# Frikallo/parakeet.cpp

Measured on AMD Instinct MI355X. Metric: RTFx (audio-sec/wall-sec), mel+encoder+TDT decode, tdt-ctc-110m 10s@b64, higher is better.
Workload: dtype f32; 1 GPU; tdt-ctc-110m, batch=64x10s clips per GPU, TDT greedy decode (the loops of 4 consecutive steps driven as one lock-step batch), fp32 (BASELINE configs[1]); parallelism=dp1 (utterance shards, no data-path collective), decode_group=4, decode_loop=phases, decode_overlap=1

## Files before the change

parakeet.cpp_amd/csrc/kernels/gemm.hip:

```cpp
#include "../pk_devmath.h"
#include "kernels.hpp"
#include <cstdio>
#include <cstdlib>
#include "gemm_pipe.hpp"
#include "gemm_bf16.hpp"
#include "gemm_bf16_glds.hpp"

namespace pk {

typedef float f32x16 __attribute__((ext_vector_type(16)));

static constexpr int BK = 32;
static constexpr int LDP = BK + 1;

template <int BM, int BN, int EPI>
__global__ __launch_bounds__(256) void gemm_nt_kernel(GemmArgs g, int tiles_n, int n_tiles) {
    constexpr int WM = BM / 2, WN = BN / 2;
    constexpr int TM = WM / 32, TN = WN / 32;
    constexpr int A_CH = BM * 8 / 256, W_CH = BN * 8 / 256;
    constexpr int NOUT = (EPI == EPI_GLU) ? BN / 2 : BN;
    static_assert(EPI != EPI_GLU || (TN % 2 == 0), "GLU needs an even number of column tiles per wave");
    extern __shared__ __attribute__((aligned(16))) float smem[];

    int bid = blockIdx.x;
    {
        const int q = n_tiles >> 3, r = n_tiles & 7, xcd = bid & 7, idx = bid >> 3;
        bid = (xcd < r ? xcd * (q + 1) : r * (q + 1) + (xcd - r) * q) + idx;
    }
    const int tile_m = bid / tiles_n, tile_n = bid % tiles_n;
    const int m0 = tile_m * BM, n0 = tile_n * NOUT;
    const int tid = threadIdx.x, lane = tid & 63, wave = tid >> 6;
    const int wm = wave >> 1, wn = wave & 1;

    const float *a_src[A_CH];
    const float *w_src[W_CH];
#pragma unroll
    for (int i = 0; i < A_CH; ++i) {
        const int c = tid + 256 * i, row = c >> 3, c4 = c & 7;
        int gr = m0 + row;
        gr = gr < g.M ? gr : g.M - 1;
        a_src[i] = g.A + (int64_t)gr * g.lda + c4 * 4;
    }
#pragma unroll
    for (int i = 0; i < W_CH; ++i) {
        const int c = tid + 256 * i, v = c >> 3, c4 = c & 7;
        int wr;
        if constexpr (EPI == EPI_GLU) {
            constexpr int HT = TN / 2;
            const int vw = v / WN, rem = v % WN, tn = rem >> 5, cc = rem & 31;
            int col = n0 + vw * (WN / 2) + (tn % HT) * 32 + cc;
            col = col < g.N ? col : g.N - 1;
            wr = (tn / HT) * g.N + col;
        } else {
            wr = n0 + v;
            wr = wr < g.N ? wr : g.N - 1;
        }
        w_src[i] = g.W + (int64_t)wr * g.ldw + c4 * 4;
    }

    float4 ra[A_CH], rw[W_CH];
    auto gload = [&](int kt) {
#pragma unroll
        for (int i = 0; i < A_CH; ++i) ra[i] = *reinterpret_cast<const float4 *>(a_src[i] + kt * BK);
#pragma unroll
        for (int i = 0; i < W_CH; ++i) rw[i] = *reinterpret_cast<const float4 *>(w_src[i] + kt * BK);
    };
    auto lstore = [&](int buf) {
        float *As = smem + buf * (BM + BN) * LDP;
        float *Ws = As + BM * LDP;
#pragma unroll
        for (int i = 0; i < A_CH; ++i) {
            const int c = tid + 256 * i;
            float *d = As + (c >> 3) * LDP + (c & 7) * 4;
            d[0] = ra[i].x; d[1] = ra[i].y; d[2] = ra[i].z; d[3] = ra[i].w;
        }
#pragma unroll
        for (int i = 0; i < W_CH; ++i) {
            const int c = tid + 256 * i;
            float *d = Ws + (c >> 3) * LDP + (c & 7) * 4;
            d[0] = rw[i].x; d[1] = rw[i].y; d[2] = rw[i].z; d[3] = rw[i].w;
        }
    };

    f32x16 acc[TM][TN];
#pragma unroll
    for (int i = 0; i < TM; ++i)
#pragma unroll
        for (int j = 0; j < TN; ++j)
#pragma unroll
            for (int r = 0; r < 16; ++r) acc[i][j][r] = 0.0f;

    const int nk = g.K / BK;
    gload(0);
    lstore(0);
    __syncthreads();
    const int frag = (lane & 31) * LDP + (lane >> 5);
    for (int kt = 0; kt < nk; ++kt) {
        const int cur = kt & 1;
        if (kt + 1 < nk) gload(kt + 1);
        const float *Ab = smem + cur * (BM + BN) * LDP + wm * WM * LDP + frag;
        const float *Wb = smem + cur * (BM + BN) * LDP + BM * LDP + wn * WN * LDP + frag;
#pragma unroll
        for (int kk = 0; kk < BK / 2; ++kk) {
            float a[TM], b[TN];
#pragma unroll
            for (int i = 0; i < TM; ++i) a[i] = Ab[i * 32 * LDP + 2 * kk];
#pragma unroll
            for (int j = 0; j < TN; ++j) b[j] = Wb[j * 32 * LDP + 2 * kk];
#pragma unroll
            for (int i = 0; i < TM; ++i)
#pragma unroll
                for (int j = 0; j < TN; ++j)
                    acc[i][j] = __builtin_amdgcn_mfma_f32_32x32x2f32(a[i], b[j], acc[i][j], 0, 0, 0);
        }
        if (kt + 1 < nk) lstore(cur ^ 1);
        __syncthreads();
    }

    const int lc = lane & 31, lr = 4 * (lane >> 5);
    constexpr int TNO = (EPI == EPI_GLU) ? TN / 2 : TN;
#pragma unroll
    for (int j = 0; j < TNO; ++j) {
        const int col = n0 + wn * (EPI == EPI_GLU ? WN / 2 : WN) + j * 32 + lc;
        if (col >= g.N) continue;
        const float bias = g.bias ? g.bias[col] : 0.0f;
        float bias_g = 0.0f;
        if constexpr (EPI == EPI_GLU) bias_g = g.bias ? g.bias[g.N + col] : 0.0f;
#pragma unroll
        for (int i = 0; i < TM; ++i) {
#pragma unroll
            for (int r = 0; r < 16; ++r) {
                const int row = m0 + wm * WM + i * 32 + (r & 3) + 8 * (r >> 2) + lr;
                if (row >= g.M) continue;
                float v = acc[i][j][r];
                if (g.bias) v = v + bias;
                if constexpr (EPI == EPI_RELU) {
                    v = v > 0.0f ? v : 0.0f;
                } else if constexpr (EPI == EPI_SILU) {
                    v = dsiluf(v);
                } else if constexpr (EPI == EPI_RESID) {
                    const float y = v * g.alpha;
                    v = g.resid[(int64_t)row * g.ldr + col] + y;
                } else if constexpr (EPI == EPI_GLU) {
                    float gt = acc[i][j + TN / 2][r];
                    if (g.bias) gt = gt + bias_g;
                    v = v * dsigmoidf(gt);
                }
                if (g.remap_rows) g.out[(int64_t)(row / g.remap_rows) * g.remap_gs + (int64_t)(row % g.remap_rows) * g.remap_rs + (int64_t)col * g.remap_cs] = v;
                else g.out[(int64_t)row * g.ldo + (col < g.sigma_cols ? ((col & ~15) | ((col & 3) << 2) | ((col >> 2) & 3)) : col)] = v;
            }
        }
    }
}

template <int BM, int BN, int EPI>
static void launch_one(const GemmArgs &a, hipStream_t s) {
    constexpr int NOUT = (EPI == EPI_GLU) ? BN / 2 : BN;
    const int tiles_m = (a.M + BM - 1) / BM, tiles_n = (a.N + NOUT - 1) / NOUT;
    const int n_tiles = tiles_m * tiles_n;
    constexpr size_t lds = 2 * (size_t)(BM + BN) * LDP * sizeof(float);
    static DynLdsSlots slots;
    ensure_dyn_lds(slots, reinterpret_cast<const void *>(&gemm_nt_kernel<BM, BN, EPI>), lds);
    hipLaunchKernelGGL((gemm_nt_kernel<BM, BN, EPI>), dim3(n_tiles), dim3(256), lds, s, a, tiles_n, n_tiles);
}

template <int EPI>
static void launch_epi(const GemmArgs &a, hipStream_t s) {
    if (a.K < 64) { launch_one<64, 64, EPI>(a, s); return; }
    const int64_t tiles128 = (int64_t)((a.M + 127) / 128) * ((a.N + 127) / 128);
    if (a.M >= 1024 && a.N >= 256 && a.K >= 1024 && a.K % 64 == 0 && tiles128 <= 256) { launch_gemm_pipe<2, 4, 2, 1, 32, EPI, 1>(a, s); return; }
    if constexpr (EPI == EPI_NONE || EPI == EPI_RELU || EPI == EPI_SILU) {
        if (a.ln_stats) { launch_gemm_pipe<4, 2, 1, 2, 32, EPI, 1, true>(a, s); return; }
    }
    if (a.M >= 1024 && (a.N >= 1024 || (a.M >= 65536 && a.N >= 256))) launch_gemm_pipe<4, 2, 1, 2, 32, EPI, 1>(a, s);
    else if (a.M >= 1024 && a.N >= 256 && a.K >= 1024) launch_gemm_pipe<2, 2, 2, 1, 32, EPI>(a, s);
    else if (a.M >= 1024 && a.N >= 256) launch_gemm_pipe<4, 2, 1, 2, 32, EPI, 1>(a, s);
    else launch_gemm_pipe<2, 2, 1, 1, 32, EPI>(a, s);
}

void launch_gemm_smallm(const GemmArgs &a, int epi, hipStream_t s);

bool gemm_ln_stats_applies(const GemmArgs &a, int epi) {
    if (!a.ln_g || !a.ln_b || !a.ln_stats || a.a_bf16 || a.out_bf16 || a.fast_act || a.a_sigma || a.W_sig) return false;
    if (a.M <= kSmallMRows || a.K < 64 || a.K % 32 != 0 || (a.lda & 3) != 0 || (a.ldw & 3) != 0) return false;
    if (epi == EPI_GLU) return true;
    if (epi != EPI_NONE && epi != EPI_RELU && epi != EPI_SILU) return false;
    const int64_t tiles128 = (int64_t)((a.M + 127) / 128) * ((a.N + 127) / 128);
    if (a.K >= 1024 && a.K % 64 == 0 && tiles128 <= 256 && a.N >= 256) return false;
    return a.M >= 1024 && a.N >= 1024;
}

void launch_gemm(const GemmArgs &a, int epi, hipStream_t s) {
    if (a.ln_stats && !gemm_ln_stats_applies(a, epi)) { fprintf(stderr, "parakeet_amd: internal error: GemmArgs::ln_stats on a product the tile kernel does not fold it into\n"); abort(); }
    if (a.M <= kSmallMRows && a.K % 64 == 0) { launch_gemm_smallm(a, epi, s); return; }
    switch (epi) {
    case EPI_NONE: launch_epi<EPI_NONE>(a, s); break;
    case EPI_RELU: launch_epi<EPI_RELU>(a, s); break;
    case EPI_SILU: launch_epi<EPI_SILU>(a, s); break;
    case EPI_RESID: launch_epi<EPI_RESID>(a, s); break;
    case EPI_GLU:
        if (a.K < 64) launch_one<128, 128, EPI_GLU>(a, s);
        else if (a.ln_stats) launch_gemm_pipe<4, 2, 1, 2, 32, EPI_GLU, 1, true>(a, s);
        else launch_gemm_pipe<4, 2, 1, 2, 32, EPI_GLU, 1>(a, s);
        break;
    default: break;
    }
}


static bool bf16_glds_rule(int M, int N, int K) {
    return M >= 8192 && N >= 512 && K >= 128 && (int64_t)N * K >= (int64_t)1024 * 1024 && (N & 3) == 0;
}
bool gemm_bf16_blocked_handoff(int M, int N, int K, int epi, bool producer) {
    if (!bf16_glds_rule(M, N, K) || (N % 16) != 0 || (K % 64) != 0) return false;
    if (!producer) return true;
    return epi != EPI_RESID && (int64_t)(M + 31) * N < ((int64_t)1 << 31);
}
[[noreturn]] static void bf16_layout_bug(const char *what) {
    fprintf(stderr, "parakeet_amd: internal error: %s (GemmArgs::out_blocked / a_blocked on a kernel that does not implement it)\n", what);
    abort();
}

template <int EPI, bool A16>
static void launch_bf16_epi(const GemmArgs &a, hipStream_t s) {
    if constexpr (A16) {
        if (a.M >= 8192 && a.N >= 512 && a.K >= 128 && (a.lda % 8) == 0 && (a.ldw % 8) == 0 && a.remap_rows == 0 && (a.ldo & 3) == 0 && (a.N & 3) == 0 &&
            (int64_t)a.N * a.K >= (int64_t)1024 * 1024) {
            constexpr int NOUT = (EPI == EPI_GLU) ? 128 : 256;
            auto est = [&](int R) {
                const int64_t tiles = (int64_t)((a.M + R - 1) / R) * ((a.N + NOUT - 1) / NOUT);
                return (double)((tiles + 255) / 256) * ((double)R * a.K * 1.008e-4 + 12.0);
            };
            if (est(192) < est(256)) launch_gemm_bf16_glds<2, 4, 3, 2, EPI>(a, s);
            else launch_gemm_bf16_glds<4, 2, 2, 4, EPI>(a, s);
            return;
        }
    }
    if (a.out_blocked || a.a_blocked) bf16_layout_bug("blocked activation layout requested for the register-staged bf16 kernel");
    if constexpr (EPI == EPI_GLU) {
        launch_gemm_bf16_t<4, 2, 1, 2, EPI_GLU, A16>(a, s);
    } else {
        if (a.M >= 1024 && (a.N >= 1024 || (a.M >= 65536 && a.N >= 256))) launch_gemm_bf16_t<4, 2, 1, 2, EPI, A16>(a, s);
        else if (a.M >= 1024 && a.N >= 256) launch_gemm_bf16_t<2, 2, 2, 1, EPI, A16>(a, s);
        else launch_gemm_bf16_t<2, 2, 1, 1, EPI, A16>(a, s);
    }
}
template <bool A16>
static void launch_gemm_bf16_a(const GemmArgs &a, int epi, hipStream_t s) {
    switch (epi) {
    case EPI_NONE: launch_bf16_epi<EPI_NONE, A16>(a, s); break;
    case EPI_RELU: launch_bf16_epi<EPI_RELU, A16>(a, s); break;
    case EPI_SILU: launch_bf16_epi<EPI_SILU, A16>(a, s); break;
    case EPI_RESID: launch_bf16_epi<EPI_RESID, A16>(a, s); break;
    case EPI_GLU: launch_bf16_epi<EPI_GLU, A16>(a, s); break;
    default: break;
    }
}
void launch_gemm_bf16(const GemmArgs &a, int epi, hipStream_t s) {
    if (gemm_smallm_bf16_applies(a, epi)) { launch_gemm_smallm_bf16(a, epi, s); return; }
    if (a.a_bf16) launch_gemm_bf16_a<true>(a, epi, s);
    else launch_gemm_bf16_a<false>(a, epi, s);
}

double gemm_flops(const GemmArgs &a, int epi) {
    return 2.0 * (double)a.M * (double)a.N * (double)a.K * (epi == EPI_GLU ? 2.0 : 1.0);
}

}
```

parakeet.cpp_amd/csrc/kernels/gemm_pipe.hpp:

```cpp
#ifndef PK_GEMM_PIPE_HPP
#define PK_GEMM_PIPE_HPP
#include <cstdio>
#include <cstdlib>
#include "../pk_devmath.h"
#include "kernels.hpp"

namespace pk {

typedef float gp_f32x16 __attribute__((ext_vector_type(16)));

template <int WGM, int WGN, int TM, int TN, int EPI, int CAP_FLOATS, bool RS_PER_PASS = false, bool EXACT = false>
__device__ __forceinline__ void gp_epilogue(const GemmArgs &g_, gp_f32x16 (&acc)[TM][TN], float *smem, int m0, int n0) {
    struct Flags { int fast_act, out_bf16; };
    const Flags gf{EXACT ? 0 : g_.fast_act, EXACT ? 0 : g_.out_bf16};
    const GemmArgs &g = g_;
    constexpr int NT = 64 * WGM * WGN;
    constexpr int WM = TM * 32, WN = TN * 32, BM = WGM * WM, BN = WGN * WN;
    constexpr int NOUT = (EPI == EPI_GLU) ? BN / 2 : BN;
    const int tid = threadIdx.x, lane = tid & 63, wave = tid >> 6;
    const int wm = wave / WGN, wn = wave % WGN;
    auto epilogue_scalar = [&](int m0, int n0) {
        const int lc = lane & 31, lr = 4 * (lane >> 5);
        constexpr int TNO = (EPI == EPI_GLU) ? TN / 2 : TN;
#pragma unroll
        for (int j = 0; j < TNO; ++j) {
            const int col = n0 + wn * (EPI == EPI_GLU ? WN / 2 : WN) + j * 32 + lc;
            if (col >= g.N) continue;
            const float bias = g.bias ? g.bias[col] : 0.0f;
            float bias_g = 0.0f;
            if constexpr (EPI == EPI_GLU) bias_g = g.bias ? g.bias[g.N + col] : 0.0f;
#pragma unroll
            for (int i = 0; i < TM; ++i) {
#pragma unroll
                for (int r = 0; r < 16; ++r) {
                    const int row = m0 + wm * WM + i * 32 + (r & 3) + 8 * (r >> 2) + lr;
                    if (row >= g.M) continue;
                    float v = acc[i][j][r];
                    if (g.bias) v = v + bias;
                    if constexpr (EPI == EPI_RELU) {
                        v = v > 0.0f ? v : 0.0f;
                    } else if constexpr (EPI == EPI_SILU) {
                        v = gf.fast_act ? fast_siluf(v) : dsiluf(v);
                    } else if constexpr (EPI == EPI_RESID) {
                        const float y = v * g.alpha;
                        v = g.resid[(int64_t)row * g.ldr + col] + y;
                    } else if constexpr (EPI == EPI_GLU) {
                        float gt = acc[i][j + TN / 2][r];
                        if (g.bias) gt = gt + bias_g;
                        v = v * (gf.fast_act ? fast_sigmoidf(gt) : dsigmoidf(gt));
                    }
                    if (g.remap_rows) g.out[(int64_t)(row / g.remap_rows) * g.remap_gs + (int64_t)(row % g.remap_rows) * g.remap_rs + (int64_t)col * g.remap_cs] = v;
                    else g.out[(int64_t)row * g.ldo + (col < g.sigma_cols ? ((col & ~15) | ((col & 3) << 2) | ((col >> 2) & 3)) : col)] = v;
                }
            }
        }
    };
    auto epilogue_wide = [&](int m0, int n0) {
        constexpr int CP = BN + 4;
        constexpr size_t CAP = (size_t)CAP_FLOATS;
        constexpr int NPASS = ((size_t)BM * CP <= CAP) ? 1 : ((size_t)BM / 2 * CP <= CAP && (BM / 2) % 32 == 0) ? 2 : ((size_t)BM / 4 * CP <= CAP && (BM / 4) % 32 == 0) ? 4
                              : ((size_t)BM / 8 * CP <= CAP && (BM / 8) % 32 == 0) ? 8 : BM / 32, PR = BM / NPASS;
        static_assert((size_t)PR * CP <= CAP, "C tile band must fit in the staging buffers");
        static_assert(PR % 32 == 0, "row bands are whole MFMA tiles");
        constexpr int C4 = NOUT / 4, NCH = BM * C4 / NT, RSTEP = NT / C4;
        static_assert((BM * C4) % NT == 0 && NT % C4 == 0, "output tile must split evenly over the threads");
        static_assert(NPASS == 1 || PR % RSTEP == 0, "row bands must split evenly over the threads' row stride");
        const int c4 = tid % C4, rl0 = tid / C4;
        const int col0 = n0 + 4 * c4;
        const bool col_ok = col0 < g.N;
        const bool sig = col0 < g.sigma_cols;
        const int blk = (4 * c4) & ~15, sa = c4 & 3;
        float bs[4] = {0.0f, 0.0f, 0.0f, 0.0f}, bg[4] = {0.0f, 0.0f, 0.0f, 0.0f};
        if (g.bias && col_ok) {
#pragma unroll
            for (int e = 0; e < 4; ++e) {
                bs[e] = g.bias[sig ? n0 + blk + 4 * e + sa : col0 + e];
                if constexpr (EPI == EPI_GLU) bg[e] = g.bias[g.N + col0 + e];
            }
        }
        constexpr int NRS = RS_PER_PASS ? NCH / NPASS : NCH;
        static_assert(!RS_PER_PASS || NCH % NPASS == 0, "chunks must split evenly over the passes");
        float4 rs[NRS];
        if constexpr (EPI == EPI_RESID && !RS_PER_PASS) {
#pragma unroll
            for (int q = 0; q < NCH; ++q) {
                int row = m0 + rl0 + q * RSTEP;
                row = row < g.M ? row : g.M - 1;
                rs[q] = col_ok ? *reinterpret_cast<const float4 *>(g.resid + (int64_t)row * g.ldr + col0) : make_float4(0.0f, 0.0f, 0.0f, 0.0f);
            }
        }
#pragma unroll
        for (int pass = 0; pass < NPASS; ++pass) {
        if constexpr (EPI == EPI_RESID && RS_PER_PASS) {
#pragma unroll
            for (int q = 0; q < NRS; ++q) {
                int row = m0 + rl0 + (pass * NRS + q) * RSTEP;
                row = row < g.M ? row : g.M - 1;
                rs[q] = col_ok ? *reinterpret_cast<const float4 *>(g.resid + (int64_t)row * g.ldr + col0) : make_float4(0.0f, 0.0f, 0.0f, 0.0f);
            }
        }
        __syncthreads();
        {
            const int lc = lane & 31, lr = 4 * (lane >> 5);
#pragma unroll
            for (int i = 0; i < TM; ++i) {
                const int rb = wm * WM + i * 32;
                if (rb / PR != pass) continue;
#pragma unroll
                for (int j = 0; j < TN; ++j)
#pragma unroll
                    for (int r = 0; r < 16; ++r)
                        smem[(rb - pass * PR + (r & 3) + 8 * (r >> 2) + lr) * CP + wn * WN + j * 32 + lc] = acc[i][j][r];
            }
        }
        __syncthreads();
#pragma unroll
        for (int q = 0; q < NCH; ++q) {
            if ((q * RSTEP) / PR != pass) continue;
            const int rl = rl0 + q * RSTEP;
            const int row = m0 + rl;
            const int rs_ = rl - pass * PR;
            float v[4], gt[4];
            if (sig) {
#pragma unroll
                for (int e = 0; e < 4; ++e) v[e] = smem[rs_ * CP + blk + 4 * e + sa];
            } else {
                int vc = 4 * c4;
                if constexpr (EPI == EPI_GLU) vc = (vc / (WN / 2)) * WN + vc % (WN / 2);
                const float4 x = *reinterpret_cast<const float4 *>(smem + rs_ * CP + vc);
                v[0] = x.x; v[1] = x.y; v[2] = x.z; v[3] = x.w;
                if constexpr (EPI == EPI_GLU) {
                    const float4 y = *reinterpret_cast<const float4 *>(smem + rs_ * CP + vc + WN / 2);
                    gt[0] = y.x; gt[1] = y.y; gt[2] = y.z; gt[3] = y.w;
                }
            }
            float rsv[4] = {0.0f, 0.0f, 0.0f, 0.0f};
            if constexpr (EPI == EPI_RESID) { const float4 &rr = rs[RS_PER_PASS ? q - pass * NRS : q]; rsv[0] = rr.x; rsv[1] = rr.y; rsv[2] = rr.z; rsv[3] = rr.w; }
            if (g.bias) {
#pragma unroll
                for (int e = 0; e < 4; ++e) {
                    v[e] = v[e] + bs[e];
                    if constexpr (EPI == EPI_GLU) gt[e] = gt[e] + bg[e];
                }
            }
            if constexpr (EPI == EPI_RELU) {
#pragma unroll
                for (int e = 0; e < 4; ++e) v[e] = v[e] > 0.0f ? v[e] : 0.0f;
            } else if constexpr (EPI == EPI_SILU) {
                if (gf.fast_act) {
#pragma unroll
                    for (int e = 0; e < 4; ++e) v[e] = fast_siluf(v[e]);
                } else {
                    dsilu4(v);
                }
            } else if constexpr (EPI == EPI_RESID) {
#pragma unroll
                for (int e = 0; e < 4; ++e) { const float y = v[e] * g.alpha; v[e] = rsv[e] + y; }
            } else if constexpr (EPI == EPI_GLU) {
                if (gf.fast_act) {
#pragma unroll
                    for (int e = 0; e < 4; ++e) gt[e] = fast_sigmoidf(gt[e]);
                } else {
                    dsigmoid4(gt);
                }
#pragma unroll
                for (int e = 0; e < 4; ++e) v[e] = v[e] * gt[e];
            }
            if (row < g.M && col_ok) {
                if (gf.out_bf16) {
                    typedef __bf16 bf16x4_ __attribute__((ext_vector_type(4)));
                    const bf16x4_ o = {(__bf16)v[0], (__bf16)v[1], (__bf16)v[2], (__bf16)v[3]};
                    *reinterpret_cast<bf16x4_ *>(reinterpret_cast<__bf16 *>(g.out) + (int64_t)row * g.ldo + col0) = o;
                } else {
                    *reinterpret_cast<float4 *>(g.out + (int64_t)row * g.ldo + col0) = make_float4(v[0], v[1], v[2], v[3]);
                }
            }
        }
        }
    };
    const bool wide = g.remap_rows == 0 && (g.ldo & 3) == 0 && (g.N & 3) == 0 && (EPI != EPI_RESID || (g.ldr & 3) == 0);
    if (wide) epilogue_wide(m0, n0);
    else epilogue_scalar(m0, n0);
}

template <int WGM, int WGN, int TM, int TN, int BK, int EPI, int NBUF = 2, bool LNA = false>
__global__ __launch_bounds__(64 * WGM * WGN) void gemm_pipe_kernel(GemmArgs g, int tiles_n, int n_tiles) {
    static_assert(NBUF == 1 || NBUF == 2, "LDS staging buffers");
    constexpr int NT = 64 * WGM * WGN;
    constexpr int WM = TM * 32, WN = TN * 32, BM = WGM * WM, BN = WGN * WN;
    constexpr int PITCH = BK + 4, BUF = (BM + BN) * PITCH, NSUB = BK / 8, C4R = BK / 4;
    constexpr int A_CH = BM * C4R / NT, W_CH = BN * C4R / NT;
    static_assert(BK == 32 || BK == 64, "BK");
    static_assert((BM * C4R) % NT == 0 && (BN * C4R) % NT == 0, "tile rows must split evenly over the threads");
    constexpr int NOUT = (EPI == EPI_GLU) ? BN / 2 : BN;
    static_assert(EPI != EPI_GLU || (TN % 2 == 0), "GLU needs an even number of column tiles per wave");
    extern __shared__ __attribute__((aligned(16))) float smem[];
    __builtin_amdgcn_s_setprio(3);

    const int tid = threadIdx.x, lane = tid & 63, wave = tid >> 6;
    const int wm = wave / WGN, wn = wave % WGN;
    const int nk = g.K / BK;

    auto chunk_row = [](int c) { const int rr = c / C4R; return (rr & ~7) | ((rr & 1) << 2) | ((rr >> 1) & 3); };
    const float *a_src[A_CH];
    const float *w_src[W_CH];
    int a_dst[A_CH], w_dst[W_CH];
    [[maybe_unused]] float a_mean[LNA ? A_CH : 1], a_rstd[LNA ? A_CH : 1];
    [[maybe_unused]] const float *gam_src = nullptr, *bet_src = nullptr;
    static_assert(!LNA || NT % C4R == 0, "LNA: a thread's chunks share their k offset");
#pragma unroll
    for (int i = 0; i < A_CH; ++i) {
        const int c = tid + NT * i;
        a_dst[i] = chunk_row(c) * PITCH + 2 * (c % C4R);
    }
#pragma unroll
    for (int i = 0; i < W_CH; ++i) {
        const int c = tid + NT * i;
        w_dst[i] = (BM + chunk_row(c)) * PITCH + 2 * (c % C4R);
    }
    auto remap = [&](int b) {
        const int q = n_tiles >> 3, r = n_tiles & 7, xcd = b & 7, idx = b >> 3;
        return (xcd < r ? xcd * (q + 1) : r * (q + 1) + (xcd - r) * q) + idx;
    };
    auto set_tile = [&](int t, int &m0, int &n0) {
        const int bid = remap(t);
        m0 = (bid / tiles_n) * BM;
        n0 = (bid % tiles_n) * NOUT;
#pragma unroll
        for (int i = 0; i < A_CH; ++i) {
            const int c = tid + NT * i;
            int gr = m0 + chunk_row(c);
            gr = gr < g.M ? gr : g.M - 1;
            a_src[i] = g.A + (int64_t)gr * g.lda + (c % C4R) * 4;
            if constexpr (LNA) {
                const float2 st = *reinterpret_cast<const float2 *>(g.ln_stats + 2 * (int64_t)gr);
                a_mean[i] = st.x; a_rstd[i] = st.y;
            }
        }
        if constexpr (LNA) { gam_src = g.ln_g + (tid % C4R) * 4; bet_src = g.ln_b + (tid % C4R) * 4; }
#pragma unroll
        for (int i = 0; i < W_CH; ++i) {
            const int c = tid + NT * i, v = chunk_row(c);
            int wr;
            if constexpr (EPI == EPI_GLU) {
                constexpr int HT = TN / 2;
                const int vw = v / WN, rem = v % WN, tn = rem >> 5, cc = rem & 31;
                int col = n0 + vw * (WN / 2) + (tn % HT) * 32 + cc;
                col = col < g.N ? col : g.N - 1;
                wr = (tn / HT) * g.N + col;
            } else {
                wr = n0 + v;
                wr = wr < g.N ? wr : g.N - 1;
            }
            w_src[i] = g.W + (int64_t)wr * g.ldw + (c % C4R) * 4;
        }
    };

    float4 ra[A_CH], rw[W_CH];
    [[maybe_unused]] float4 rg4, rb4;
    auto gload = [&](int kt) {
#pragma unroll
        for (int i = 0; i < A_CH; ++i) ra[i] = *reinterpret_cast<const float4 *>(a_src[i] + kt * BK);
#pragma unroll
        for (int i = 0; i < W_CH; ++i) rw[i] = *reinterpret_cast<const float4 *>(w_src[i] + kt * BK);
        if constexpr (LNA) {
            rg4 = *reinterpret_cast<const float4 *>(gam_src + kt * BK);
            rb4 = *reinterpret_cast<const float4 *>(bet_src + kt * BK);
        }
    };
    auto st2 = [&](float *p, float a, float b, float c, float d) {
        if (EPI == EPI_NONE) {
            *reinterpret_cast<float2 *>(p) = make_float2(a, b);
            *reinterpret_cast<float2 *>(p + BK / 2) = make_float2(c, d);
        } else {
            const unsigned addr = (unsigned)(size_t)p;
            asm volatile("ds_write_b32 %0, %1\n\tds_write_b32 %0, %2 offset:4\n\tds_write_b32 %0, %3 offset:%5\n\tds_write_b32 %0, %4 offset:%6"
                         ::"v"(addr), "v"(a), "v"(b), "v"(c), "v"(d), "n"(BK / 2 * 4), "n"(BK / 2 * 4 + 4) : "memory");
        }
    };
    auto lnorm = [&]() {
        if constexpr (LNA) {
            typedef float f2_ __attribute__((ext_vector_type(2)));
            const f2_ g01 = {rg4.x, rg4.y}, g23 = {rg4.z, rg4.w}, b01 = {rb4.x, rb4.y}, b23 = {rb4.z, rb4.w};
#pragma unroll
            for (int i = 0; i < A_CH; ++i) {
                const f2_ m = {a_mean[i], a_mean[i]}, r = {a_rstd[i], a_rstd[i]};
                f2_ lo = {ra[i].x, ra[i].y}, hi = {ra[i].z, ra[i].w};
                lo = __builtin_elementwise_fma((lo - m) * r, g01, b01);
                hi = __builtin_elementwise_fma((hi - m) * r, g23, b23);
                ra[i] = make_float4(lo.x, lo.y, hi.x, hi.y);
            }
        }
    };
    auto lstore = [&](int buf) {
        float *base = smem + buf * BUF;
#pragma unroll
        for (int i = 0; i < A_CH; ++i) st2(base + a_dst[i], ra[i].x, ra[i].z, ra[i].y, ra[i].w);
#pragma unroll
        for (int i = 0; i < W_CH; ++i) st2(base + w_dst[i], rw[i].x, rw[i].z, rw[i].y, rw[i].w);
    };

    gp_f32x16 acc[TM][TN];
    auto zero_acc = [&]() {
#pragma unroll
        for (int i = 0; i < TM; ++i)
#pragma unroll
            for (int j = 0; j < TN; ++j)
#pragma unroll
                for (int r = 0; r < 16; ++r) acc[i][j][r] = 0.0f;
    };

    const int fa_off = (wm * WM + (lane & 31)) * PITCH + (BK / 2) * (lane >> 5);
    const int fb_off = (BM + wn * WN + (lane & 31)) * PITCH + (BK / 2) * (lane >> 5);
    float4 fa[2][TM], fb[2][TN];
    auto fragload = [&](int buf, int s, int slot) {
        const float *base = smem + buf * BUF + 4 * s;
#pragma unroll
        for (int i = 0; i < TM; ++i) fa[slot][i] = *reinterpret_cast<const float4 *>(base + fa_off + i * 32 * PITCH);
#pragma unroll
        for (int j = 0; j < TN; ++j) fb[slot][j] = *reinterpret_cast<const float4 *>(base + fb_off + j * 32 * PITCH);
    };
    auto mma = [&](int slot) {
#pragma unroll
        for (int e = 0; e < 4; ++e) {
#pragma unroll
            for (int i = 0; i < TM; ++i) {
                const float a = e == 0 ? fa[slot][i].x : e == 1 ? fa[slot][i].y : e == 2 ? fa[slot][i].z : fa[slot][i].w;
#pragma unroll
                for (int j = 0; j < TN; ++j) {
                    const float b = e == 0 ? fb[slot][j].x : e == 1 ? fb[slot][j].y : e == 2 ? fb[slot][j].z : fb[slot][j].w;
                    acc[i][j] = __builtin_amdgcn_mfma_f32_32x32x2f32(a, b, acc[i][j], 0, 0, 0);
                }
            }
        }
    };
    auto epilogue = [&](int m0, int n0) { gp_epilogue<WGM, WGN, TM, TN, EPI, NBUF * BUF, false, true>(g, acc, smem, m0, n0); };
#define GP_SB() __builtin_amdgcn_sched_barrier(0)
#ifndef GP_LNORM_AT
#define GP_LNORM_AT (NSUB - 2)
#endif

    int m0, n0;
    set_tile(blockIdx.x, m0, n0);
    gload(0);
    lnorm();
    lstore(0);
    lds_store_fence();
    __syncthreads();
    gload(1);
    fragload(0, 0, 0);
    int cur = 0;
    zero_acc();
    if constexpr (NBUF == 1) {
        for (int kt = 0; kt < nk; ++kt) {
            const bool more1 = kt + 1 < nk, more2 = kt + 2 < nk;
#pragma unroll
            for (int s = 0; s < NSUB - 1; ++s) {
                fragload(0, s + 1, (s + 1) & 1);
                GP_SB(); mma(s & 1); GP_SB();
                if (LNA && s == GP_LNORM_AT && more1) { lnorm(); GP_SB(); }
            }
            __syncthreads();
            if (more1) lstore(0);
            if (more2) gload(kt + 2);
            GP_SB(); mma((NSUB - 1) & 1); GP_SB();
            lds_store_fence();
            __syncthreads();
            if (more1) fragload(0, 0, 0);
        }
    } else {
        for (int kt = 0; kt < nk; ++kt) {
            const bool more1 = kt + 1 < nk, more2 = kt + 2 < nk;
#pragma unroll
            for (int s = 0; s < NSUB - 1; ++s) {
                fragload(cur, s + 1, (s + 1) & 1);
                if (LNA && s == 0 && more1) lnorm();
                if (s == NSUB - 2 && more1) lstore(cur ^ 1);
                GP_SB(); mma(s & 1); GP_SB();
            }
            lds_store_fence();
            __syncthreads();
            if (more1) fragload(cur ^ 1, 0, 0);
            if (more2) gload(kt + 2);
            GP_SB(); mma((NSUB - 1) & 1); GP_SB();
            cur ^= 1;
        }
    }
    epilogue(m0, n0);
#undef GP_SB
}

template <int WGM, int WGN, int TM, int TN, int BK, int EPI, int NBUF = 2, bool LNA = false>
static void launch_gemm_pipe(const GemmArgs &a, hipStream_t s) {
    constexpr int BM = WGM * TM * 32, BN = WGN * TN * 32;
    constexpr int NOUT = (EPI == EPI_GLU) ? BN / 2 : BN;
    const int tiles_m = (a.M + BM - 1) / BM, tiles_n = (a.N + NOUT - 1) / NOUT;
    const int n_tiles = tiles_m * tiles_n;
    constexpr size_t lds = NBUF * (size_t)(BM + BN) * (BK + 4) * sizeof(float);
    if (a.fast_act || a.out_bf16) { fprintf(stderr, "parakeet_amd: internal error: bf16-mode switches on the fp32 GEMM\n"); abort(); }
    if (LNA != (a.ln_stats != nullptr)) { fprintf(stderr, "parakeet_amd: internal error: GemmArgs::ln_stats on a kernel without the folded LayerNorm (or the reverse)\n"); abort(); }
    auto kern = &gemm_pipe_kernel<WGM, WGN, TM, TN, BK, EPI, NBUF, LNA>;
    static DynLdsSlots slots;
    ensure_dyn_lds(slots, reinterpret_cast<const void *>(kern), lds);
    hipLaunchKernelGGL(kern, dim3(n_tiles), dim3(64 * WGM * WGN), lds, s, a, tiles_n, n_tiles);
}

}
#endif
```

Before: 35570 x real-time.

## Interleave LDS stores and global loads with MFMAs in single-buffered fp32 GEMM loop

Adds a SCHED template variant of the single-buffered pipelined fp32 GEMM main loop. Between the two barriers, the last k-substep's MFMAs are split per instruction and interleaved with per-chunk LDS stores and next-tile global loads. The remaining SCHED k-steps of MFMAs run after the second barrier, overlapping the first fragment load. The goal is to hide barrier and memory latency behind matrix math, at the cost of fixed scheduling barriers, longer register live ranges, and an unconditional (clamped) global load on the final iterations.

```diff
diff --git a/parakeet.cpp_amd/csrc/kernels/gemm.hip b/parakeet.cpp_amd/csrc/kernels/gemm.hip
--- a/parakeet.cpp_amd/csrc/kernels/gemm.hip
+++ b/parakeet.cpp_amd/csrc/kernels/gemm.hip
@@ -164,17 +164,18 @@
     hipLaunchKernelGGL((gemm_nt_kernel<BM, BN, EPI>), dim3(n_tiles), dim3(256), lds, s, a, tiles_n, n_tiles);
 }
 
+constexpr int kSbSched = 2;
 template <int EPI>
 static void launch_epi(const GemmArgs &a, hipStream_t s) {
     if (a.K < 64) { launch_one<64, 64, EPI>(a, s); return; }
     const int64_t tiles128 = (int64_t)((a.M + 127) / 128) * ((a.N + 127) / 128);
-    if (a.M >= 1024 && a.N >= 256 && a.K >= 1024 && a.K % 64 == 0 && tiles128 <= 256) { launch_gemm_pipe<2, 4, 2, 1, 32, EPI, 1>(a, s); return; }
+    if (a.M >= 1024 && a.N >= 256 && a.K >= 1024 && a.K % 64 == 0 && tiles128 <= 256) { launch_gemm_pipe<2, 4, 2, 1, 32, EPI, 1, false, EPI == EPI_NONE ? 0 : kSbSched>(a, s); return; }
     if constexpr (EPI == EPI_NONE || EPI == EPI_RELU || EPI == EPI_SILU) {
-        if (a.ln_stats) { launch_gemm_pipe<4, 2, 1, 2, 32, EPI, 1, true>(a, s); return; }
-    }
-    if (a.M >= 1024 && (a.N >= 1024 || (a.M >= 65536 && a.N >= 256))) launch_gemm_pipe<4, 2, 1, 2, 32, EPI, 1>(a, s);
+        if (a.ln_stats) { launch_gemm_pipe<4, 2, 1, 2, 32, EPI, 1, true, kSbSched>(a, s); return; }
+    }
+    if (a.M >= 1024 && (a.N >= 1024 || (a.M >= 65536 && a.N >= 256))) launch_gemm_pipe<4, 2, 1, 2, 32, EPI, 1, false, kSbSched>(a, s);
     else if (a.M >= 1024 && a.N >= 256 && a.K >= 1024) launch_gemm_pipe<2, 2, 2, 1, 32, EPI>(a, s);
-    else if (a.M >= 1024 && a.N >= 256) launch_gemm_pipe<4, 2, 1, 2, 32, EPI, 1>(a, s);
+    else if (a.M >= 1024 && a.N >= 256) launch_gemm_pipe<4, 2, 1, 2, 32, EPI, 1, false, kSbSched>(a, s);
     else launch_gemm_pipe<2, 2, 1, 1, 32, EPI>(a, s);
 }
 
@@ -200,8 +201,8 @@
     case EPI_RESID: launch_epi<EPI_RESID>(a, s); break;
     case EPI_GLU:
         if (a.K < 64) launch_one<128, 128, EPI_GLU>(a, s);
-        else if (a.ln_stats) launch_gemm_pipe<4, 2, 1, 2, 32, EPI_GLU, 1, true>(a, s);
-        else launch_gemm_pipe<4, 2, 1, 2, 32, EPI_GLU, 1>(a, s);
+        else if (a.ln_stats) launch_gemm_pipe<4, 2, 1, 2, 32, EPI_GLU, 1, true, kSbSched>(a, s);
+        else launch_gemm_pipe<4, 2, 1, 2, 32, EPI_GLU, 1, false, kSbSched>(a, s);
         break;
     default: break;
     }
diff --git a/parakeet.cpp_amd/csrc/kernels/gemm_pipe.hpp b/parakeet.cpp_amd/csrc/kernels/gemm_pipe.hpp
--- a/parakeet.cpp_amd/csrc/kernels/gemm_pipe.hpp
+++ b/parakeet.cpp_amd/csrc/kernels/gemm_pipe.hpp
@@ -183,9 +183,10 @@
     else epilogue_scalar(m0, n0);
 }
 
-template <int WGM, int WGN, int TM, int TN, int BK, int EPI, int NBUF = 2, bool LNA = false>
+template <int WGM, int WGN, int TM, int TN, int BK, int EPI, int NBUF = 2, bool LNA = false, int SCHED = 0>
 __global__ __launch_bounds__(64 * WGM * WGN) void gemm_pipe_kernel(GemmArgs g, int tiles_n, int n_tiles) {
     static_assert(NBUF == 1 || NBUF == 2, "LDS staging buffers");
+    static_assert(SCHED >= 0 && SCHED < 4 && (SCHED == 0 || NBUF == 1), "SCHED: 0..3 k-steps after the second barrier, single-buffered loop only");
     constexpr int NT = 64 * WGM * WGN;
     constexpr int WM = TM * 32, WN = TN * 32, BM = WGM * WM, BN = WGN * WN;
     constexpr int PITCH = BK + 4, BUF = (BM + BN) * PITCH, NSUB = BK / 8, C4R = BK / 4;
@@ -258,6 +259,10 @@
 
     float4 ra[A_CH], rw[W_CH];
     [[maybe_unused]] float4 rg4, rb4;
+    auto gload_chunk = [&](int q, int kt) {
+        if (q < A_CH) ra[q] = *reinterpret_cast<const float4 *>(a_src[q] + kt * BK);
+        else rw[q - A_CH] = *reinterpret_cast<const float4 *>(w_src[q - A_CH] + kt * BK);
+    };
     auto gload = [&](int kt) {
 #pragma unroll
         for (int i = 0; i < A_CH; ++i) ra[i] = *reinterpret_cast<const float4 *>(a_src[i] + kt * BK);
@@ -292,6 +297,10 @@
             }
         }
     };
+    auto lstore_chunk = [&](int q) {
+        if (q < A_CH) st2(smem + a_dst[q], ra[q].x, ra[q].z, ra[q].y, ra[q].w);
+        else st2(smem + w_dst[q - A_CH], rw[q - A_CH].x, rw[q - A_CH].z, rw[q - A_CH].y, rw[q - A_CH].w);
+    };
     auto lstore = [&](int buf) {
         float *base = smem + buf * BUF;
 #pragma unroll
@@ -333,6 +342,11 @@
                 }
             }
         }
+    };
+    auto mma_one = [&](int slot, int e, int i, int j) {
+        const float a = e == 0 ? fa[slot][i].x : e == 1 ? fa[slot][i].y : e == 2 ? fa[slot][i].z : fa[slot][i].w;
+        const float b = e == 0 ? fb[slot][j].x : e == 1 ? fb[slot][j].y : e == 2 ? fb[slot][j].z : fb[slot][j].w;
+        acc[i][j] = __builtin_amdgcn_mfma_f32_32x32x2f32(a, b, acc[i][j], 0, 0, 0);
     };
     auto epilogue = [&](int m0, int n0) { gp_epilogue<WGM, WGN, TM, TN, EPI, NBUF * BUF, false, true>(g, acc, smem, m0, n0); };
 #define GP_SB() __builtin_amdgcn_sched_barrier(0)
@@ -351,7 +365,47 @@
     fragload(0, 0, 0);
     int cur = 0;
     zero_acc();
-    if constexpr (NBUF == 1) {
+    if constexpr (NBUF == 1 && SCHED > 0) {
+        constexpr int NCH = A_CH + W_CH, E1 = 4 - SCHED, M1 = E1 * TM * TN;
+        for (int kt = 0; kt < nk; ++kt) {
+            const bool more1 = kt + 1 < nk;
+            const int kl = kt + 2 < nk ? kt + 2 : nk - 1;
+#pragma unroll
+            for (int s = 0; s < NSUB - 1; ++s) {
+                fragload(0, s + 1, (s + 1) & 1);
+                GP_SB(); mma(s & 1); GP_SB();
+                if (LNA && s == GP_LNORM_AT && more1) { lnorm(); GP_SB(); }
+            }
+            constexpr int SL = (NSUB - 1) & 1;
+            __syncthreads();
+            GP_SB();
+#pragma unroll
+            for (int q = 0; q < M1; ++q) {
+                const int e = q / (TM * TN), i = (q / TN) % TM, j = q % TN;
+                mma_one(SL, e, i, j);
+                GP_SB();
+#pragma unroll
+                for (int c = q * NCH / M1; c < (q + 1) * NCH / M1; ++c) { lstore_chunk(c); GP_SB(); gload_chunk(c, kl); GP_SB(); }
+            }
+            if constexpr (LNA) {
+                rg4 = *reinterpret_cast<const float4 *>(gam_src + kl * BK);
+                rb4 = *reinterpret_cast<const float4 *>(bet_src + kl * BK);
+                GP_SB();
+            }
+            lds_store_fence();
+            __syncthreads();
+            GP_SB();
+            fragload(0, 0, 0);
+            GP_SB();
+#pragma unroll
+            for (int e = E1; e < 4; ++e)
+#pragma unroll
+                for (int i = 0; i < TM; ++i)
+#pragma unroll
+                    for (int j = 0; j < TN; ++j) mma_one(SL, e, i, j);
+            GP_SB();
+        }
+    } else if constexpr (NBUF == 1) {
         for (int kt = 0; kt < nk; ++kt) {
             const bool more1 = kt + 1 < nk, more2 = kt + 2 < nk;
 #pragma unroll
@@ -390,7 +444,7 @@
 #undef GP_SB
 }
 
-template <int WGM, int WGN, int TM, int TN, int BK, int EPI, int NBUF = 2, bool LNA = false>
+template <int WGM, int WGN, int TM, int TN, int BK, int EPI, int NBUF = 2, bool LNA = false, int SCHED = 0>
 static void launch_gemm_pipe(const GemmArgs &a, hipStream_t s) {
     constexpr int BM = WGM * TM * 32, BN = WGN * TN * 32;
     constexpr int NOUT = (EPI == EPI_GLU) ? BN / 2 : BN;
@@ -399,7 +453,7 @@
     constexpr size_t lds = NBUF * (size_t)(BM + BN) * (BK + 4) * sizeof(float);
     if (a.fast_act || a.out_bf16) { fprintf(stderr, "parakeet_amd: internal error: bf16-mode switches on the fp32 GEMM\n"); abort(); }
     if (LNA != (a.ln_stats != nullptr)) { fprintf(stderr, "parakeet_amd: internal error: GemmArgs::ln_stats on a kernel without the folded LayerNorm (or the reverse)\n"); abort(); }
-    auto kern = &gemm_pipe_kernel<WGM, WGN, TM, TN, BK, EPI, NBUF, LNA>;
+    auto kern = &gemm_pipe_kernel<WGM, WGN, TM, TN, BK, EPI, NBUF, LNA, SCHED>;
     static DynLdsSlots slots;
     ensure_dyn_lds(slots, reinterpret_cast<const void *>(kern), lds);
     hipLaunchKernelGGL(kern, dim3(n_tiles), dim3(64 * WGM * WGN), lds, s, a, tiles_n, n_tiles);
```

Measured after the change: 36140 x real-time, median of 6. 1.6% higher.
